# jrl-umi3218/jrl-walkgen

Hardware: NVIDIA B200
Metric: Kajita preview steps/s (batched; Herdt2010 QP solves/s reported under 'herdt') (higher is better)
Workload: dtype f64

## Files before the change

jrl_walkgen_b200/csrc/preview.cu:

```cuda
#include "wg_common.h"
#include <atomic>
#include <mutex>
#include <cstdlib>
#include <vector>
#include <cmath>
#include <algorithm>
#include <type_traits>

#define WG_HD __host__ __device__

namespace {

struct Mat {
  int n;
  double a[16];
  WG_HD double &operator()(int i, int j) { return a[i * n + j]; }
  WG_HD double operator()(int i, int j) const { return a[i * n + j]; }
};

WG_HD Mat mat_zero(int n)
{
  Mat C;
  C.n = n;
  for (int i = 0; i < 16; ++i) C.a[i] = 0.0;
// ... 229 lines not shown
constexpr int SCAN_LEVELS = 6;

struct PreviewConsts {
  double A[9], B[3], C[3], Kx[3], Ks;
  int NL, NLpad;
  double P[2][SCAN_LEVELS][16];
  double G[2][FIR_R][4], H[2][FIR_R][4];
  double RF0[FIR_R], RFN[FIR_R];
  double RV[FIR_R][4], RVN[FIR_R][4];
  double RW[FIR_R + 1][4];
  double RP[SCAN_LEVELS][16];
};
__constant__ PreviewConsts c_pc;
__constant__ double c_F[WG_PREVIEW_MAX_NL + 8];

namespace {
struct PreviewImage {
  PreviewConsts pc;
  double F[WG_PREVIEW_MAX_NL + 8];
};
std::mutex g_pv_mutex;
std::atomic<unsigned long long> g_pv_gen_counter{0};
unsigned long long g_pv_bound[64];

int preview_bind(wg_ctx *ctx)
{
  if (ctx->device < 0 || ctx->device >= 64) return WG_ERR_INVALID;
  if (g_pv_bound[ctx->device] == ctx->preview_gen) return WG_OK;
  const PreviewImage *im = reinterpret_cast<const PreviewImage *>(ctx->preview_image.data());
  WG_CUDA(ctx, cudaDeviceSynchronize());
  WG_CUDA(ctx, cudaMemcpyToSymbol(c_pc, &im->pc, sizeof im->pc));
  WG_CUDA(ctx, cudaMemcpyToSymbol(c_F, im->F, sizeof im->F));
  g_pv_bound[ctx->device] = ctx->preview_gen;
  return WG_OK;
}
}

constexpr int PV_MAX_CHUNKS = 16;

struct wg_preview_plan {
  wg_ctx *ctx;
  int B;
  int NL;
  int64_t total_samples, total_steps;
  int64_t *d_offsets;
  int *d_order;
  double *d_zmp, *d_state, *d_com, *d_zmpout, *d_add;
  int n_chunks;
  int chunk_first[PV_MAX_CHUNKS + 1];
  int64_t chunk_samp[PV_MAX_CHUNKS + 1];
  int *d_order_chunked;
  cudaStream_t up_stream, down_stream;
  cudaEvent_t ev_up[PV_MAX_CHUNKS], ev_k[PV_MAX_CHUNKS], ev_done;
};

__device__ __forceinline__ int pad9(int e) { return e + (e >> 3); }
__device__ __forceinline__ int swz8(int e) { return e ^ ((e >> 3) & 7); }

struct Axis {
  double x0, x1, x2, s;
};
template <bool SIM>
__device__ __forceinline__ double preview_tick(Axis &a, double f, double pk)
{
  double r = c_pc.Kx[0] * a.x0;
  r = fma(c_pc.Kx[1], a.x1, r);
  r = fma(c_pc.Kx[2], a.x2, r);
  const double u = fma(c_pc.Ks, a.s, -r) + f;
  const double n0 = fma(c_pc.A[2], a.x2, fma(c_pc.A[1], a.x1, a.x0));
  const double n1 = fma(c_pc.A[5], a.x2, a.x1);
  a.x0 = fma(u, c_pc.B[0], n0);
  a.x1 = fma(u, c_pc.B[1], n1);
  a.x2 = fma(u, c_pc.B[2], a.x2);
  const double z = fma(c_pc.C[2], a.x2, fma(c_pc.C[1], a.x1, c_pc.C[0] * a.x0));
  if (SIM) a.s += (pk - z);
  return z;
}

__device__ __forceinline__ Axis axis_zero()
{
  Axis a;
  a.x0 = a.x1 = a.x2 = a.s = 0.0;
  return a;
}
__device__ __forceinline__ void operator+=(Axis &a, const Axis &b)
{
  a.x0 += b.x0; a.x1 += b.x1; a.x2 += b.x2; a.s += b.s;
}
__device__ __forceinline__ void axpy(Axis &c, const double *g, double a)
{
  c.x0 = fma(g[0], a, c.x0); c.x1 = fma(g[1], a, c.x1);
  c.x2 = fma(g[2], a, c.x2); c.s = fma(g[3], a, c.s);
}
__device__ __forceinline__ Axis shfl_up(const Axis &a, int d)
{
  Axis r;
  r.x0 = __shfl_up_sync(0xffffffffu, a.x0, d); r.x1 = __shfl_up_sync(0xffffffffu, a.x1, d);
  r.x2 = __shfl_up_sync(0xffffffffu, a.x2, d); r.s = __shfl_up_sync(0xffffffffu, a.s, d);
  return r;
}
__device__ __forceinline__ Axis shfl_down(const Axis &a, int d)
{
  Axis r;
  r.x0 = __shfl_down_sync(0xffffffffu, a.x0, d); r.x1 = __shfl_down_sync(0xffffffffu, a.x1, d);
  r.x2 = __shfl_down_sync(0xffffffffu, a.x2, d); r.s = __shfl_down_sync(0xffffffffu, a.s, d);
  return r;
// ... 501 lines not shown
            if (ADD) {
              double q[12];
              ld32g(ga + 6 * r0, q[0], q[1], q[2], q[3], c32);
              ld32g(ga + 6 * r0 + 4, q[4], q[5], q[6], q[7], c32);
              ld32g(ga + 6 * r0 + 8, q[8], q[9], q[10], q[11], c32);
              a0 += q[0]; a1 += q[1]; a2 += q[2]; a3 += q[3]; a4 += q[4]; a5 += q[5];
              b0 += q[6]; b1 += q[7]; b2 += q[8]; b3 += q[9]; b4 += q[10]; b5 += q[11];
            }
            st32g(gc + 6 * r0, a0, a1, a2, a3, c32);
            st32g(gc + 6 * r0 + 4, a4, a5, b0, b1, c32);
            st32g(gc + 6 * r0 + 8, b2, b3, b4, b5, c32);
          }
          if (zmp) st32g(gz + 2 * r0, u0, u1, POS ? sx.x0 : zx1, POS ? sy.x0 : zy1, z32);
        } else if (k0 + r0 <= last) {
          const double zx0 = preview_tick<SIM>(sx, ax[r0], pk[r0].x);
          const double zy0 = preview_tick<SIM>(sy, ay[r0], pk[r0].y);
          if (com) {
            double a0 = sx.x0, a1 = sx.x1, a2 = sx.x2, a3 = sy.x0, a4 = sy.x1, a5 = sy.x2;
            if (ADD) {
              const double2 q0 = __ldg(reinterpret_cast<const double2 *>(ga + 6 * r0));
              const double2 q1 = __ldg(reinterpret_cast<const double2 *>(ga + 6 * r0) + 1);
              const double2 q2 = __ldg(reinterpret_cast<const double2 *>(ga + 6 * r0) + 2);
              a0 += q0.x; a1 += q0.y; a2 += q1.x; a3 += q1.y; a4 += q2.x; a5 += q2.y;
            }
            double2 *g2 = reinterpret_cast<double2 *>(gc + 6 * r0);
            g2[0] = make_double2(a0, a1); g2[1] = make_double2(a2, a3); g2[2] = make_double2(a4, a5);
          }
          if (zmp) *reinterpret_cast<double2 *>(gz + 2 * r0) = POS ? make_double2(sx.x0, sy.x0) : make_double2(zx0, zy0);
        }
      }
    }
    if (k0 <= last && last < k0 + FIR_R) store_state(s_carry, sx, sy);
    base += FIR_TILE;
    if (base >= CAP) base -= CAP;
  }
  __syncthreads();
  if (t < 8) state[8 * (size_t)b + t] = s_carry[t];
}

constexpr int RW_TILE = FIR_R * 32;
constexpr int RW_U = 5;

__device__ __forceinline__ void bulk_store(double *dst, unsigned src_smem, unsigned bytes)
{
  asm volatile("cp.async.bulk.global.shared::cta.bulk_group [%0], [%1], %2;\n" ::"l"(dst), "r"(src_smem), "r"(bytes) : "memory");
}
__device__ __forceinline__ bool elect_one()
{
  unsigned r;
  asm volatile("{\n .reg .pred p;\n elect.sync _|p, 0xffffffff;\n selp.u32 %0, 1, 0, p;\n}\n" : "=r"(r));
  return r != 0;
}

template <bool SIM, bool ADD = false, bool POS = false>
__global__ void __launch_bounds__(32, 10)
preview_rec_warp_kernel(const int *__restrict__ order, const int64_t *__restrict__ offsets,
                        const double2 *__restrict__ p, double *__restrict__ state, double *__restrict__ com,
                        double *__restrict__ zmp, const double *__restrict__ com_add, const double2 *__restrict__ Etab)
{
  constexpr unsigned FULL = 0xffffffffu;
  extern __shared__ double2 sp[];
  __shared__ double s_halo[8];
  __shared__ double s_carry[8];
  const int b = order[blockIdx.x];
  const int64_t o = offsets[b];
  const int L = (int)(offsets[b + 1] - o);
  const int NL = c_pc.NL, NLpad = c_pc.NLpad;
  const int nsteps = L - NL + 1;
  if (nsteps <= 0) return;
  const int lane = threadIdx.x;
  const int CAP = RW_TILE + NLpad;
  double2 *stage = sp + CAP + 25 * lane;
  if (lane < 8) s_carry[lane] = state[8 * (size_t)b + lane];
  const double(*Pm)[16] = c_pc.P[SIM ? 1 : 0];
  const double2 *src = p + o;
  for (int e = lane; e < CAP; e += 32) cp_async16(sp + swz8(e), src + (e < L ? e : 0), e < L ? 16u : 0u);
  cp_async_commit();
  int base = 0;

  for (int start = 0; start < nsteps; start += RW_TILE) {
    cp_async_wait_all();
    __syncwarp();
    int own0 = base + FIR_R * lane;
    if (own0 >= CAP) own0 -= CAP;

    {
      double h[8];
#pragma unroll
      for (int j = 0; j < 8; ++j) h[j] = 0.0;
      int hb = base + RW_TILE;
      if (hb >= CAP) hb -= CAP;
      for (int i0 = lane; i0 < NL; i0 += 32 * RW_U) {
        double2 e01[RW_U], e23[RW_U], q[RW_U];
#pragma unroll
        for (int u = 0; u < RW_U; ++u) {
          const int i = i0 + 32 * u;
          const bool in = i < NL;
          const int ii = in ? i : 0;
          ld32g(reinterpret_cast<const double *>(Etab + 2 * ii), e01[u].x, e01[u].y, e23[u].x, e23[u].y, true);
          int hi = hb + ii;
          if (hi >= CAP) hi -= CAP;
          q[u] = in ? sp[swz8(hi)] : make_double2(0.0, 0.0);
        }
#pragma unroll
        for (int u = 0; u < RW_U; ++u) {
          h[0] = fma(e01[u].x, q[u].x, h[0]); h[1] = fma(e01[u].y, q[u].x, h[1]);
          h[2] = fma(e23[u].x, q[u].x, h[2]); h[3] = fma(e23[u].y, q[u].x, h[3]);
          h[4] = fma(e01[u].x, q[u].y, h[4]); h[5] = fma(e01[u].y, q[u].y, h[5]);
          h[6] = fma(e23[u].x, q[u].y, h[6]); h[7] = fma(e23[u].y, q[u].y, h[7]);
        }
      }
      double k4[4], k2[2], k1;
      {
        const bool up = (lane & 16) != 0;
#pragma unroll
        for (int j = 0; j < 4; ++j) {
          const double send = up ? h[j] : h[4 + j];
          k4[j] = (up ? h[4 + j] : h[j]) + __shfl_xor_sync(FULL, send, 16);
        }
      }
      {
        const bool up = (lane & 8) != 0;
#pragma unroll
        for (int j = 0; j < 2; ++j) {
          const double send = up ? k4[j] : k4[2 + j];
          k2[j] = (up ? k4[2 + j] : k4[j]) + __shfl_xor_sync(FULL, send, 8);
        }
      }
      {
        const bool up = (lane & 4) != 0;
        const double send = up ? k2[0] : k2[1];
        k1 = (up ? k2[1] : k2[0]) + __shfl_xor_sync(FULL, send, 4);
      }
      k1 += __shfl_xor_sync(FULL, k1, 2);
      k1 += __shfl_xor_sync(FULL, k1, 1);
      if ((lane & 3) == 0) s_halo[((lane & 16) ? 4 : 0) + ((lane & 8) ? 2 : 0) + ((lane & 4) ? 1 : 0)] = k1;
    }

    double ax[FIR_R], ay[FIR_R];
    double2 pk[FIR_R];
    Axis bx, by;
    {
      const double2 *own = sp + own0;
      const int osw = (own0 >> 3) & 7;
      local_pass<SIM>([&](int j) { return own[j ^ osw]; }, [&](int i) { return sp[swz8(i)]; }, own0, NL, CAP, ax, ay, pk, bx, by);
    }
    __syncwarp();
    if (start + RW_TILE < nsteps) {
      const int first = start + CAP;
#pragma unroll
      for (int u = 0; u < FIR_R; ++u) {
        const int e = lane + 32 * u;
        int ri = base + e;
        if (ri >= CAP) ri -= CAP;
        const bool in = first + e < L;
        cp_async16(sp + swz8(ri), src + (in ? first + e : 0), in ? 16u : 0u);
      }
      cp_async_commit();
    }
    Axis ix, iy;
    load_pair(s_halo, ix, iy);
    if (lane == 31) {
      scan_combine(bx, c_pc.RP[0], ix);
      scan_combine(by, c_pc.RP[0], iy);
    }
    scan_down(bx, by, lane);
    {
      const Axis a = shfl_down(bx, 1), b = shfl_down(by, 1);
      if (lane != 31) { ix = a; iy = b; }
    }
    add_window(ax, ay, ix, iy);

    Axis cx, cy, inx, iny;
    local_aggregate<SIM>(ax, ay, pk, lane == 0, s_carry, Pm, cx, cy, inx, iny);
    scan_up(cx, cy, lane, Pm);
    Axis sx = shfl_up(cx, 1), sy = shfl_up(cy, 1);
    if (lane == 0) { sx = inx; sy = iny; }
    __syncwarp();
    const int k0 = start + FIR_R * lane;
    const int last = min(start + RW_TILE, nsteps) - 1;
    {
      double *gc = com ? com + 6 * (size_t)(o + k0) : nullptr;
      double *gz = zmp ? zmp + 2 * (size_t)(o + k0) : nullptr;
      const double *ga = ADD ? com_add + 6 * (size_t)(o + k0) : nullptr;
      const bool c32 = ((reinterpret_cast<uintptr_t>(gc) | (ADD ? reinterpret_cast<uintptr_t>(ga) : 0)) & 31) == 0;
      const bool z32 = (reinterpret_cast<uintptr_t>(gz) & 31) == 0;
      const bool bulk = com != nullptr;
      if (bulk) {
        asm volatile("cp.async.bulk.wait_group.read 0;\n" ::: "memory");
        __syncwarp();
      }
#pragma unroll
      for (int j = 0; j < FIR_R / 2; ++j) {
        const int r0 = 2 * j, r1 = 2 * j + 1;
        if (k0 + r1 <= last) {
          const double zx0 = preview_tick<SIM>(sx, ax[r0], pk[r0].x);
          const double zy0 = preview_tick<SIM>(sy, ay[r0], pk[r0].y);
          double a0 = sx.x0, a1 = sx.x1, a2 = sx.x2, a3 = sy.x0, a4 = sy.x1, a5 = sy.x2;
          const double u0 = POS ? sx.x0 : zx0, u1 = POS ? sy.x0 : zy0;
          const double zx1 = preview_tick<SIM>(sx, ax[r1], pk[r1].x);
          const double zy1 = preview_tick<SIM>(sy, ay[r1], pk[r1].y);
          if (com) {
            double b0 = sx.x0, b1 = sx.x1, b2 = sx.x2, b3 = sy.x0, b4 = sy.x1, b5 = sy.x2;
            if (ADD) {
              double q[12];
              ld32g(ga + 6 * r0, q[0], q[1], q[2], q[3], c32);
              ld32g(ga + 6 * r0 + 4, q[4], q[5], q[6], q[7], c32);
              ld32g(ga + 6 * r0 + 8, q[8], q[9], q[10], q[11], c32);
              a0 += q[0]; a1 += q[1]; a2 += q[2]; a3 += q[3]; a4 += q[4]; a5 += q[5];
              b0 += q[6]; b1 += q[7]; b2 += q[8]; b3 += q[9]; b4 += q[10]; b5 += q[11];
            }
            if (bulk) {
              double2 *sg = stage + 6 * j;
              sg[0] = make_double2(a0, a1); sg[1] = make_double2(a2, a3); sg[2] = make_double2(a4, a5);
              sg[3] = make_double2(b0, b1); sg[4] = make_double2(b2, b3); sg[5] = make_double2(b4, b5);
            } else {
              st32g(gc + 6 * r0, a0, a1, a2, a3, c32);
              st32g(gc + 6 * r0 + 4, a4, a5, b0, b1, c32);
              st32g(gc + 6 * r0 + 8, b2, b3, b4, b5, c32);
            }
          }
          if (zmp) st32g(gz + 2 * r0, u0, u1, POS ? sx.x0 : zx1, POS ? sy.x0 : zy1, z32);
        } else if (k0 + r0 <= last) {
          const double zx0 = preview_tick<SIM>(sx, ax[r0], pk[r0].x);
          const double zy0 = preview_tick<SIM>(sy, ay[r0], pk[r0].y);
          if (com) {
            double a0 = sx.x0, a1 = sx.x1, a2 = sx.x2, a3 = sy.x0, a4 = sy.x1, a5 = sy.x2;
            if (ADD) {
              const double2 q0 = __ldg(reinterpret_cast<const double2 *>(ga + 6 * r0));
              const double2 q1 = __ldg(reinterpret_cast<const double2 *>(ga + 6 * r0) + 1);
              const double2 q2 = __ldg(reinterpret_cast<const double2 *>(ga + 6 * r0) + 2);
              a0 += q0.x; a1 += q0.y; a2 += q1.x; a3 += q1.y; a4 += q2.x; a5 += q2.y;
            }
            double2 *g2 = reinterpret_cast<double2 *>(gc + 6 * r0);
            g2[0] = make_double2(a0, a1); g2[1] = make_double2(a2, a3); g2[2] = make_double2(a4, a5);
          }
          if (zmp) *reinterpret_cast<double2 *>(gz + 2 * r0) = POS ? make_double2(sx.x0, sy.x0) : make_double2(zx0, zy0);
        }
      }
      if (bulk) {
        asm volatile("fence.proxy.async.shared::cta;\n" ::: "memory");
        __syncwarp();
        if (elect_one()) {
          const int nt = last - start + 1;
          double *g = com + 6 * (size_t)(o + start);
          const unsigned sa = (unsigned)__cvta_generic_to_shared(sp + CAP);
          if (nt >= RW_TILE) {
#pragma unroll
            for (int i = 0; i < 32; ++i) bulk_store(g + 6 * FIR_R * i, sa + 400u * i, 96u * (FIR_R / 2));
          } else {
            for (int i = 0; i < 32 && FIR_R * i + 1 < nt; ++i)
              bulk_store(g + 6 * FIR_R * i, sa + 400u * i, 96u * (unsigned)min(FIR_R / 2, (nt - FIR_R * i) / 2));
          }
          asm volatile("cp.async.bulk.commit_group;\n" ::: "memory");
        }
      }
    }
    if (k0 <= last && last < k0 + FIR_R) store_state(s_carry, sx, sy);
    base += RW_TILE;
    if (base >= CAP) base -= CAP;
  }
  __syncwarp();
  asm volatile("cp.async.bulk.wait_group 0;\n" ::: "memory");
  if (lane < 8) state[8 * (size_t)b + lane] = s_carry[lane];
}

namespace {

void scan_matrices(const wg_preview_gains_t &g, bool sim, double (*P)[16], double (*G)[4], double (*H)[4])
{
  typedef long double LD;
  LD M[4][4];
  for (int j = 0; j < 4; ++j) {
    LD x[3] = {0, 0, 0}, s = 0;
    if (j < 3) x[j] = 1; else s = 1;
    const LD u = (LD)g.Ks * s - ((LD)g.Kx[0] * x[0] + (LD)g.Kx[1] * x[1] + (LD)g.Kx[2] * x[2]);
    LD n[3];
    for (int i = 0; i < 3; ++i)
      n[i] = (LD)g.A[3 * i] * x[0] + (LD)g.A[3 * i + 1] * x[1] + (LD)g.A[3 * i + 2] * x[2] + (LD)g.B[i] * u;
    const LD z = (LD)g.C[0] * n[0] + (LD)g.C[1] * n[1] + (LD)g.C[2] * n[2];
    for (int i = 0; i < 3; ++i) M[i][j] = n[i];
    M[3][j] = sim ? s - z : s;
  }
  auto square = [](LD X[4][4]) {
    LD Y[4][4];
    for (int i = 0; i < 4; ++i)
      for (int j = 0; j < 4; ++j) {
        LD a = 0;
        for (int k = 0; k < 4; ++k) a += X[i][k] * X[k][j];
        Y[i][j] = a;
      }
    std::memcpy(X, Y, sizeof Y);
  };
  if (G && H) {
    LD g4[4], h4[4] = {0, 0, 0, 0};
    LD zb = 0;
    for (int i = 0; i < 3; ++i) { g4[i] = (LD)g.B[i]; zb += (LD)g.C[i] * (LD)g.B[i]; }
    g4[3] = sim ? -zb : (LD)0;
    h4[3] = sim ? (LD)1 : (LD)0;
    for (int r = FIR_R - 1; r >= 0; --r) {
      for (int i = 0; i < 4; ++i) { G[r][i] = (double)g4[i]; H[r][i] = (double)h4[i]; }
      LD gn[4], hn[4];
      for (int i = 0; i < 4; ++i) {
        gn[i] = 0; hn[i] = 0;
        for (int k = 0; k < 4; ++k) { gn[i] += M[i][k] * g4[k]; hn[i] += M[i][k] * h4[k]; }
      }
      std::memcpy(g4, gn, sizeof gn); std::memcpy(h4, hn, sizeof hn);
    }
  }
  for (int r = 1; r < FIR_R; r <<= 1) square(M);
  for (int l = 0; l < SCAN_LEVELS; ++l) {
    for (int i = 0; i < 4; ++i)
      for (int j = 0; j < 4; ++j) P[l][4 * i + j] = (double)M[i][j];
    square(M);
  }
}

// ... 117 lines not shown
    std::memcpy(Pl, P8, sizeof Pl);
    for (int l = 0; l < SCAN_LEVELS; ++l) {
      for (int i = 0; i < 4; ++i) for (int j = 0; j < 4; ++j) pc.RP[l][4 * i + j] = (double)Pl[i][j];
      mul(Pl, Pl, Pl);
    }
    LD Pm[4][4];
    for (int i = 0; i < 4; ++i) for (int j = 0; j < 4; ++j) Pm[i][j] = (i == j) ? 1 : 0;
    double *lp = tables.data() + (size_t)NLpad * 4;
    for (int m = 0; m < 32; ++m) {
      for (int i = 0; i < 4; ++i) for (int j = 0; j < 4; ++j) lp[16 * m + 4 * i + j] = (double)Pm[i][j];
      mul(P8, Pm, Pm);
    }
  }
  return (double)(res / tot);
}

}

template <class... P, class... A>
static int preview_launch(wg_ctx *ctx, void (*kern)(P...), int count, int threads, size_t smem, const char *too_large,
                          A... args)
{
  if (smem > 96 * 1024) return wg_fail(ctx, WG_ERR_INVALID, too_large);
  std::lock_guard<std::mutex> lock(g_pv_mutex);
  { const int rc = preview_bind(ctx); if (rc != WG_OK) return rc; }
  WG_SMEM_ATTR(ctx, kern, smem);
  wg_prof_start(ctx, WG_K_PREVIEW_FUSED);
  kern<<<count, threads, smem, ctx->stream>>>(args...);
  wg_prof_stop(ctx);
  WG_LAUNCHED(ctx);
  return WG_OK;
}

template <bool SIM, bool ADD, bool POS>
static int preview_launch_variant(wg_ctx *ctx, wg_preview_plan *pl, bool recursive, int shape, const int *d_order, int count,
                                  const double2 *pz, double *d_state, double *d_com, double *d_zmpout, const double *d_com_add)
{
  const int NLpad = (pl->NL + FIR_R - 1) / FIR_R * FIR_R;
  const int64_t *off = pl->d_offsets;
  if (!recursive) {
    auto smem = [&](int threads) {
      const int span = FIR_R * threads + NLpad;
      return sizeof(double2) * std::max<size_t>((size_t)(span + (span >> 3) + 2), (size_t)(threads / 32) * 320);
    };
    const char *msg = "preview window too large for the FIR tile";
    switch (shape) {
    case 1: return preview_launch(ctx, preview_fused_kernel<SIM, 128, 4, ADD, POS>, count, 128, smem(128), msg, d_order, off, pz, d_state, d_com, d_zmpout, d_com_add);
    case 2: return preview_launch(ctx, preview_fused_kernel<SIM, 32, 16, ADD, POS>, count, 32, smem(32), msg, d_order, off, pz, d_state, d_com, d_zmpout, d_com_add);
    default: return preview_launch(ctx, preview_fused_kernel<SIM, 64, 8, ADD, POS>, count, 64, smem(64), msg, d_order, off, pz, d_state, d_com, d_zmpout, d_com_add);
    }
  }
  const double2 *E = reinterpret_cast<const double2 *>(ctx->preview_rec_dev);
  const char *msg = "preview window too large for the tile";
  if (shape == 2)
    return preview_launch(ctx, preview_rec_warp_kernel<SIM, ADD, POS>, count, 32, sizeof(double2) * (size_t)(RW_TILE + NLpad + 25 * 32),
                          msg, d_order, off, pz, d_state, d_com, d_zmpout, d_com_add, E);
  auto smem = [&](int threads) {
    const int cap = 2 * FIR_R * threads + NLpad;
    return sizeof(double2) * (size_t)(cap + (cap >> 3) + 2);
  };
  const double2 *lp = E + 2 * (size_t)NLpad;
  switch (shape) {
  case 1: return preview_launch(ctx, preview_rec_kernel<SIM, 128, 4, ADD, POS>, count, 128, smem(128), msg, d_order, off, pz, d_state, d_com, d_zmpout, d_com_add, E, lp);
  case 3: return preview_launch(ctx, preview_rec_kernel<SIM, 256, 2, ADD, POS>, count, 256, smem(256), msg, d_order, off, pz, d_state, d_com, d_zmpout, d_com_add, E, lp);
  default: return preview_launch(ctx, preview_rec_kernel<SIM, 64, 8, ADD, POS>, count, 64, smem(64), msg, d_order, off, pz, d_state, d_com, d_zmpout, d_com_add, E, lp);
  }
}

extern "C" {

int wg_preview_set_gains(wg_ctx *ctx, const wg_preview_gains_t *g)
{
  if (!ctx || !g || g->NL <= 0 || g->NL > WG_PREVIEW_MAX_NL) return WG_ERR_INVALID;
  wg_device_guard guard(ctx->device);
  static_assert((FIR_R & (FIR_R - 1)) == 0, "FIR_R must be a power of two");
  ctx->preview_image.assign(sizeof(PreviewImage), 0);
  PreviewImage *im = reinterpret_cast<PreviewImage *>(ctx->preview_image.data());
  PreviewConsts &pc = im->pc;
  std::memcpy(pc.A, g->A, sizeof pc.A);
  std::memcpy(pc.B, g->B, sizeof pc.B);
  std::memcpy(pc.C, g->C, sizeof pc.C);
  std::memcpy(pc.Kx, g->Kx, sizeof pc.Kx);
  pc.Ks = g->Ks;
  pc.NL = g->NL;
  pc.NLpad = (g->NL + FIR_R - 1) / FIR_R * FIR_R;
  scan_matrices(*g, false, pc.P[0], pc.G[0], pc.H[0]);
  scan_matrices(*g, true, pc.P[1], pc.G[1], pc.H[1]);
  std::copy(g->F, g->F + g->NL, im->F);
  {
    std::vector<double> tables;
    ctx->preview_rec_residual = rec_setup(*g, pc, tables);
    ctx->preview_rec_ok = ctx->preview_rec_residual >= 0.0 && ctx->preview_rec_residual <= WG_PREVIEW_REC_TOL;
    if (ctx->preview_rec_dev) { WG_CUDA(ctx, cudaStreamSynchronize(ctx->stream)); cudaFree(ctx->preview_rec_dev); ctx->preview_rec_dev = nullptr; }
    if (ctx->preview_rec_ok) {
      WG_CUDA(ctx, cudaMalloc(&ctx->preview_rec_dev, sizeof(double) * tables.size()));
      WG_CUDA(ctx, cudaMemcpy(ctx->preview_rec_dev, tables.data(), sizeof(double) * tables.size(), cudaMemcpyHostToDevice));
    }
  }
  ctx->preview_gains = *g;
  ctx->preview_gen = ++g_pv_gen_counter;
  ctx->preview_ready = true;
  return WG_OK;
}

double wg_preview_sum_fit(const wg_preview_gains_t *g)
{
  if (!g || g->NL <= 0 || g->NL > WG_PREVIEW_MAX_NL) return -1.0;
  PreviewConsts pc;
  std::vector<double> tables;
// ... 38 lines not shown
{
  if (!ctx) return WG_ERR_INVALID;
  if (!ctx->preview_ready) return wg_fail(ctx, WG_ERR_NOT_READY, "wg_preview_set_gains not called");
  if (mode_in_use)
    *mode_in_use = (ctx->preview_sum_mode != WG_PREVIEW_SUM_DIRECT && ctx->preview_rec_ok) ? WG_PREVIEW_SUM_RECURSIVE : WG_PREVIEW_SUM_DIRECT;
  if (fit_residual) *fit_residual = ctx->preview_rec_residual;
  return WG_OK;
}

int wg_preview_plan_create(wg_ctx *ctx, int B, const int64_t *offsets, wg_preview_plan **out)
{
  if (!ctx || !out || B < 0 || (B > 0 && !offsets)) return WG_ERR_INVALID;
  if (!ctx->preview_ready) return wg_fail(ctx, WG_ERR_NOT_READY, "wg_preview_set_gains not called");
  wg_device_guard guard(ctx->device);
  *out = nullptr;
  const int NL = ctx->preview_gains.NL;
  if (B > 0 && offsets[0] != 0) return wg_fail(ctx, WG_ERR_INVALID, "offsets[0] must be 0");
  int64_t total_steps = 0;
  std::vector<int> order(B);
  for (int b = 0; b < B; ++b) {
    const int64_t L = offsets[b + 1] - offsets[b];
    if (L < 0 || L > 0x3fffffff) return wg_fail(ctx, WG_ERR_INVALID, "offsets must be non-decreasing");
    if (L >= NL) total_steps += L - NL + 1;
    order[b] = b;
  }
  std::stable_sort(order.begin(), order.end(), [&](int a, int b) {
    return offsets[a + 1] - offsets[a] > offsets[b + 1] - offsets[b];
  });
  wg_preview_plan *pl = new (std::nothrow) wg_preview_plan();
  if (!pl) return WG_ERR_ALLOC;
  std::memset(pl, 0, sizeof *pl);
  pl->ctx = ctx; pl->B = B; pl->NL = NL;
  pl->total_samples = B > 0 ? offsets[B] : 0;
  pl->total_steps = total_steps;
  pl->n_chunks = std::max(1, std::min(PV_MAX_CHUNKS, B / 8));
  {
    const int64_t total = B > 0 ? offsets[B] : 0;
    int b = 0;
    pl->chunk_first[0] = 0;
    for (int c = 1; c < pl->n_chunks; ++c) {
      const int64_t target = total * c / pl->n_chunks;
      while (b < B && offsets[b] < target) ++b;
      pl->chunk_first[c] = std::max(b, pl->chunk_first[c - 1]);
    }
    pl->chunk_first[pl->n_chunks] = B;
    for (int c = 0; c <= pl->n_chunks; ++c) pl->chunk_samp[c] = B > 0 ? offsets[pl->chunk_first[c]] : 0;
  }
  std::vector<int> order_chunked(B);
  for (int b = 0; b < B; ++b) order_chunked[b] = b;
  for (int c = 0; c < pl->n_chunks; ++c)
    std::stable_sort(order_chunked.begin() + pl->chunk_first[c], order_chunked.begin() + pl->chunk_first[c + 1], [&](int a, int b) {
      return offsets[a + 1] - offsets[a] > offsets[b + 1] - offsets[b];
    });
  cudaError_t e = cudaMalloc(&pl->d_offsets, sizeof(int64_t) * (B + 1));
  if (e == cudaSuccess) e = cudaMalloc(&pl->d_order, sizeof(int) * std::max(1, B));
  if (e == cudaSuccess) e = cudaMalloc(&pl->d_order_chunked, sizeof(int) * std::max(1, B));
  if (e == cudaSuccess && B > 0)
    e = cudaMemcpyAsync(pl->d_order_chunked, order_chunked.data(), sizeof(int) * B, cudaMemcpyHostToDevice, ctx->stream);
  if (e == cudaSuccess) e = cudaStreamCreateWithFlags(&pl->up_stream, cudaStreamNonBlocking);
  if (e == cudaSuccess) e = cudaStreamCreateWithFlags(&pl->down_stream, cudaStreamNonBlocking);
  for (int c = 0; c < PV_MAX_CHUNKS && e == cudaSuccess; ++c) {
    e = cudaEventCreateWithFlags(&pl->ev_up[c], cudaEventDisableTiming);
    if (e == cudaSuccess) e = cudaEventCreateWithFlags(&pl->ev_k[c], cudaEventDisableTiming);
  }
  if (e == cudaSuccess) e = cudaEventCreateWithFlags(&pl->ev_done, cudaEventDisableTiming);
  if (e == cudaSuccess && B > 0)
    e = cudaMemcpyAsync(pl->d_offsets, offsets, sizeof(int64_t) * (B + 1), cudaMemcpyHostToDevice, ctx->stream);
  if (e == cudaSuccess && B > 0)
    e = cudaMemcpyAsync(pl->d_order, order.data(), sizeof(int) * B, cudaMemcpyHostToDevice, ctx->stream);
  if (e == cudaSuccess) e = cudaStreamSynchronize(ctx->stream);
  if (e != cudaSuccess) {
    wg_fail(ctx, WG_ERR_CUDA, "wg_preview_plan_create", e);
    wg_preview_plan_destroy(pl);
    return WG_ERR_CUDA;
  }
  *out = pl;
  return WG_OK;
}

int wg_preview_plan_destroy(wg_preview_plan *pl)
{
  if (!pl) return WG_OK;
  wg_device_guard guard(pl->ctx->device);
  cudaStreamSynchronize(pl->ctx->stream);
  if (pl->up_stream) { cudaStreamSynchronize(pl->up_stream); cudaStreamDestroy(pl->up_stream); }
  if (pl->down_stream) { cudaStreamSynchronize(pl->down_stream); cudaStreamDestroy(pl->down_stream); }
  for (int c = 0; c < PV_MAX_CHUNKS; ++c) { if (pl->ev_up[c]) cudaEventDestroy(pl->ev_up[c]); if (pl->ev_k[c]) cudaEventDestroy(pl->ev_k[c]); }
  if (pl->ev_done) cudaEventDestroy(pl->ev_done);
  cudaFree(pl->d_offsets); cudaFree(pl->d_order); cudaFree(pl->d_order_chunked);
  cudaFree(pl->d_zmp); cudaFree(pl->d_state); cudaFree(pl->d_com); cudaFree(pl->d_zmpout); cudaFree(pl->d_add);
  delete pl;
  return WG_OK;
}

int wgi_preview_plan_set_offsets(wg_preview_plan *pl, const int64_t *offsets_host)
{
  wg_ctx *ctx = pl->ctx;
  int64_t total_steps = 0;
  for (int b = 0; b < pl->B; ++b) {
    const int64_t L = offsets_host[b + 1] - offsets_host[b];
    if (L >= pl->NL) total_steps += L - pl->NL + 1;
  }
  pl->total_samples = pl->B > 0 ? offsets_host[pl->B] : 0;
  pl->total_steps = total_steps;
  if (pl->B > 0)
    WG_CUDA(ctx, cudaMemcpyAsync(pl->d_offsets, offsets_host, sizeof(int64_t) * (pl->B + 1), cudaMemcpyHostToDevice, ctx->stream));
  return WG_OK;
}

int64_t wg_preview_plan_total_steps(const wg_preview_plan *pl) { return pl ? pl->total_steps : 0; }
int64_t wg_preview_plan_total_samples(const wg_preview_plan *pl) { return pl ? pl->total_samples : 0; }

int wgi_preview_launch_range(wg_ctx *ctx, wg_preview_plan *pl, const int *d_order, int count, const double *d_zmp,
                            double *d_state, double *d_com, double *d_zmpout, int simulation, const double *d_com_add,
                            int pos_only)
{
  if (pl->total_steps == 0 || count <= 0) return WG_OK;
  static int forced = -2;
  if (forced == -2) {
    const char *e = getenv("WG_PREVIEW_SHAPE");
    forced = e ? atoi(e) : -1;
  }
  const bool recursive = ctx->preview_sum_mode != WG_PREVIEW_SUM_DIRECT && ctx->preview_rec_ok;
  int shape = forced >= 0 ? forced : ctx->preview_cta_shape >= 0 ? ctx->preview_cta_shape : !recursive ? 0 : count >= 1792 ? 2 : count >= 768 ? 1 : 3;
  if (shape == 3) {
    const int NLpad = (pl->NL + FIR_R - 1) / FIR_R * FIR_R, cap = 2 * FIR_R * 256 + NLpad;
    if (!recursive || sizeof(double2) * (size_t)(cap + (cap >> 3) + 2) > 96 * 1024) shape = 1;
  }
  if (ctx->preview_sum_mode == WG_PREVIEW_SUM_RECURSIVE && !ctx->preview_rec_ok)
    return wg_fail(ctx, WG_ERR_INVALID, "WG_PREVIEW_SUM_RECURSIVE: the window weights of this context are not of the form w' L^i v");
  const double2 *pz = reinterpret_cast<const double2 *>(d_zmp);
  auto launch = [&](auto sim, auto add, auto pos) {
    return preview_launch_variant<sim, add, pos>(ctx, pl, recursive, shape, d_order, count, pz, d_state, pos ? nullptr : d_com,
                                                 d_zmpout, add ? d_com_add : nullptr);
  };
  const std::true_type T{};
  const std::false_type F{};
  if (pos_only) return simulation ? launch(T, F, T) : launch(F, F, T);
  if (d_com_add && d_com) return launch(T, T, F);
  return simulation ? launch(T, F, F) : launch(F, F, F);
}

// ... 212 lines not shown
```

Before: 50.64 billion.

## Make warp preview kernel persistent with atomic ticket work-stealing across walks

Converts the one-warp-per-walk preview kernel into a persistent kernel launched with as many blocks as fit resident on the GPU. Each warp takes walk indices from a global atomic ticket counter and prefetches the next walk's first window while finishing the current one. The tile body is factored into a helper with refill and carry callbacks. This is meant to cut per-block launch and scheduling overhead and to overlap the next walk's load with the current tail. The cost is an atomic per walk and a monotonically growing ticket counter kept on the host.

```diff
diff --git a/jrl_walkgen_b200/csrc/preview.cu b/jrl_walkgen_b200/csrc/preview.cu
--- a/jrl_walkgen_b200/csrc/preview.cu
+++ b/jrl_walkgen_b200/csrc/preview.cu
@@ -305,6 +305,9 @@
   int *d_order_chunked;
   cudaStream_t up_stream, down_stream;
   cudaEvent_t ev_up[PV_MAX_CHUNKS], ev_k[PV_MAX_CHUNKS], ev_done;
+  unsigned long long *d_next;
+  unsigned long long tickets;
+  int resident;
 };
 
 __device__ __forceinline__ int pad9(int e) { return e + (e >> 3); }
@@ -912,217 +915,262 @@
   return r != 0;
 }
 
+template <bool SIM, bool ADD, bool POS, class Refill, class CarryIn, class CarryOut>
+__device__ __forceinline__ void rec_warp_tile(double2 *sp, double *s_halo, int lane, int CAP, int base, int start, int nsteps,
+                                              int64_t o, double *com, double *zmp, const double *com_add, const double2 *Etab,
+                                              Refill refill, CarryIn carry_in, CarryOut carry_out)
+{
+  constexpr unsigned FULL = 0xffffffffu;
+  const int NL = c_pc.NL;
+  const double(*Pm)[16] = c_pc.P[SIM ? 1 : 0];
+  double2 *stage = sp + CAP + 25 * lane;
+  int own0 = base + FIR_R * lane;
+  if (own0 >= CAP) own0 -= CAP;
+
+  {
+    double h[8];
+#pragma unroll
+    for (int j = 0; j < 8; ++j) h[j] = 0.0;
+    int hb = base + RW_TILE;
+    if (hb >= CAP) hb -= CAP;
+    for (int i0 = lane; i0 < NL; i0 += 32 * RW_U) {
+      double2 e01[RW_U], e23[RW_U], q[RW_U];
+#pragma unroll
+      for (int u = 0; u < RW_U; ++u) {
+        const int i = i0 + 32 * u;
+        const bool in = i < NL;
+        const int ii = in ? i : 0;
+        ld32g(reinterpret_cast<const double *>(Etab + 2 * ii), e01[u].x, e01[u].y, e23[u].x, e23[u].y, true);
+        int hi = hb + ii;
+        if (hi >= CAP) hi -= CAP;
+        q[u] = in ? sp[swz8(hi)] : make_double2(0.0, 0.0);
+      }
+#pragma unroll
+      for (int u = 0; u < RW_U; ++u) {
+        h[0] = fma(e01[u].x, q[u].x, h[0]); h[1] = fma(e01[u].y, q[u].x, h[1]);
+        h[2] = fma(e23[u].x, q[u].x, h[2]); h[3] = fma(e23[u].y, q[u].x, h[3]);
+        h[4] = fma(e01[u].x, q[u].y, h[4]); h[5] = fma(e01[u].y, q[u].y, h[5]);
+        h[6] = fma(e23[u].x, q[u].y, h[6]); h[7] = fma(e23[u].y, q[u].y, h[7]);
+      }
+    }
+    double k4[4], k2[2], k1;
+    {
+      const bool up = (lane & 16) != 0;
+#pragma unroll
+      for (int j = 0; j < 4; ++j) {
+        const double send = up ? h[j] : h[4 + j];
+        k4[j] = (up ? h[4 + j] : h[j]) + __shfl_xor_sync(FULL, send, 16);
+      }
+    }
+    {
+      const bool up = (lane & 8) != 0;
+#pragma unroll
+      for (int j = 0; j < 2; ++j) {
+        const double send = up ? k4[j] : k4[2 + j];
+        k2[j] = (up ? k4[2 + j] : k4[j]) + __shfl_xor_sync(FULL, send, 8);
+      }
+    }
+    {
+      const bool up = (lane & 4) != 0;
+      const double send = up ? k2[0] : k2[1];
+      k1 = (up ? k2[1] : k2[0]) + __shfl_xor_sync(FULL, send, 4);
+    }
+    k1 += __shfl_xor_sync(FULL, k1, 2);
+    k1 += __shfl_xor_sync(FULL, k1, 1);
+    if ((lane & 3) == 0) s_halo[((lane & 16) ? 4 : 0) + ((lane & 8) ? 2 : 0) + ((lane & 4) ? 1 : 0)] = k1;
+  }
+
+  double ax[FIR_R], ay[FIR_R];
+  double2 pk[FIR_R];
+  Axis bx, by;
+  {
+    const double2 *own = sp + own0;
+    const int osw = (own0 >> 3) & 7;
+    local_pass<SIM>([&](int j) { return own[j ^ osw]; }, [&](int i) { return sp[swz8(i)]; }, own0, NL, CAP, ax, ay, pk, bx, by);
+  }
+  __syncwarp();
+  refill();
+  Axis ix, iy;
+  load_pair(s_halo, ix, iy);
+  if (lane == 31) {
+    scan_combine(bx, c_pc.RP[0], ix);
+    scan_combine(by, c_pc.RP[0], iy);
+  }
+  scan_down(bx, by, lane);
+  {
+    const Axis a = shfl_down(bx, 1), b = shfl_down(by, 1);
+    if (lane != 31) { ix = a; iy = b; }
+  }
+  add_window(ax, ay, ix, iy);
+
+  Axis cx, cy, inx, iny;
+  {
+    double q[8];
+    const double *cin = carry_in(q);
+    local_aggregate<SIM>(ax, ay, pk, lane == 0, cin, Pm, cx, cy, inx, iny);
+  }
+  scan_up(cx, cy, lane, Pm);
+  Axis sx = shfl_up(cx, 1), sy = shfl_up(cy, 1);
+  if (lane == 0) { sx = inx; sy = iny; }
+  __syncwarp();
+  const int k0 = start + FIR_R * lane;
+  const int last = min(start + RW_TILE, nsteps) - 1;
+  {
+    double *gc = com ? com + 6 * (size_t)(o + k0) : nullptr;
+    double *gz = zmp ? zmp + 2 * (size_t)(o + k0) : nullptr;
+    const double *ga = ADD ? com_add + 6 * (size_t)(o + k0) : nullptr;
+    const bool c32 = ((reinterpret_cast<uintptr_t>(gc) | (ADD ? reinterpret_cast<uintptr_t>(ga) : 0)) & 31) == 0;
+    const bool z32 = (reinterpret_cast<uintptr_t>(gz) & 31) == 0;
+    const bool bulk = com != nullptr;
+    if (bulk) {
+      asm volatile("cp.async.bulk.wait_group.read 0;\n" ::: "memory");
+      __syncwarp();
+    }
+#pragma unroll
+    for (int j = 0; j < FIR_R / 2; ++j) {
+      const int r0 = 2 * j, r1 = 2 * j + 1;
+      if (k0 + r1 <= last) {
+        const double zx0 = preview_tick<SIM>(sx, ax[r0], pk[r0].x);
+        const double zy0 = preview_tick<SIM>(sy, ay[r0], pk[r0].y);
+        double a0 = sx.x0, a1 = sx.x1, a2 = sx.x2, a3 = sy.x0, a4 = sy.x1, a5 = sy.x2;
+        const double u0 = POS ? sx.x0 : zx0, u1 = POS ? sy.x0 : zy0;
+        const double zx1 = preview_tick<SIM>(sx, ax[r1], pk[r1].x);
+        const double zy1 = preview_tick<SIM>(sy, ay[r1], pk[r1].y);
+        if (com) {
+          double b0 = sx.x0, b1 = sx.x1, b2 = sx.x2, b3 = sy.x0, b4 = sy.x1, b5 = sy.x2;
+          if (ADD) {
+            double q[12];
+            ld32g(ga + 6 * r0, q[0], q[1], q[2], q[3], c32);
+            ld32g(ga + 6 * r0 + 4, q[4], q[5], q[6], q[7], c32);
+            ld32g(ga + 6 * r0 + 8, q[8], q[9], q[10], q[11], c32);
+            a0 += q[0]; a1 += q[1]; a2 += q[2]; a3 += q[3]; a4 += q[4]; a5 += q[5];
+            b0 += q[6]; b1 += q[7]; b2 += q[8]; b3 += q[9]; b4 += q[10]; b5 += q[11];
+          }
+          if (bulk) {
+            double2 *sg = stage + 6 * j;
+            sg[0] = make_double2(a0, a1); sg[1] = make_double2(a2, a3); sg[2] = make_double2(a4, a5);
+            sg[3] = make_double2(b0, b1); sg[4] = make_double2(b2, b3); sg[5] = make_double2(b4, b5);
+          } else {
+            st32g(gc + 6 * r0, a0, a1, a2, a3, c32);
+            st32g(gc + 6 * r0 + 4, a4, a5, b0, b1, c32);
+            st32g(gc + 6 * r0 + 8, b2, b3, b4, b5, c32);
+          }
+        }
+        if (zmp) st32g(gz + 2 * r0, u0, u1, POS ? sx.x0 : zx1, POS ? sy.x0 : zy1, z32);
+      } else if (k0 + r0 <= last) {
+        const double zx0 = preview_tick<SIM>(sx, ax[r0], pk[r0].x);
+        const double zy0 = preview_tick<SIM>(sy, ay[r0], pk[r0].y);
+        if (com) {
+          double a0 = sx.x0, a1 = sx.x1, a2 = sx.x2, a3 = sy.x0, a4 = sy.x1, a5 = sy.x2;
+          if (ADD) {
+            const double2 q0 = __ldg(reinterpret_cast<const double2 *>(ga + 6 * r0));
+            const double2 q1 = __ldg(reinterpret_cast<const double2 *>(ga + 6 * r0) + 1);
+            const double2 q2 = __ldg(reinterpret_cast<const double2 *>(ga + 6 * r0) + 2);
+            a0 += q0.x; a1 += q0.y; a2 += q1.x; a3 += q1.y; a4 += q2.x; a5 += q2.y;
+          }
+          double2 *g2 = reinterpret_cast<double2 *>(gc + 6 * r0);
+          g2[0] = make_double2(a0, a1); g2[1] = make_double2(a2, a3); g2[2] = make_double2(a4, a5);
+        }
+        if (zmp) *reinterpret_cast<double2 *>(gz + 2 * r0) = POS ? make_double2(sx.x0, sy.x0) : make_double2(zx0, zy0);
+      }
+    }
+    if (bulk) {
+      asm volatile("fence.proxy.async.shared::cta;\n" ::: "memory");
+      __syncwarp();
+      if (elect_one()) {
+        const int nt = last - start + 1;
+        double *g = com + 6 * (size_t)(o + start);
+        const unsigned sa = (unsigned)__cvta_generic_to_shared(sp + CAP);
+        if (nt >= RW_TILE) {
+#pragma unroll
+          for (int i = 0; i < 32; ++i) bulk_store(g + 6 * FIR_R * i, sa + 400u * i, 96u * (FIR_R / 2));
+        } else {
+          for (int i = 0; i < 32 && FIR_R * i + 1 < nt; ++i)
+            bulk_store(g + 6 * FIR_R * i, sa + 400u * i, 96u * (unsigned)min(FIR_R / 2, (nt - FIR_R * i) / 2));
+        }
+        asm volatile("cp.async.bulk.commit_group;\n" ::: "memory");
+      }
+    }
+  }
+  if (k0 <= last && last < k0 + FIR_R) carry_out(sx, sy);
+}
+
 template <bool SIM, bool ADD = false, bool POS = false>
 __global__ void __launch_bounds__(32, 10)
-preview_rec_warp_kernel(const int *__restrict__ order, const int64_t *__restrict__ offsets,
-                        const double2 *__restrict__ p, double *__restrict__ state, double *__restrict__ com,
-                        double *__restrict__ zmp, const double *__restrict__ com_add, const double2 *__restrict__ Etab)
+preview_rec_warp_kernel(const int *__restrict__ order, int count, unsigned long long *next, unsigned long long ticket0,
+                        const int64_t *__restrict__ offsets, const double2 *__restrict__ p, double *__restrict__ state,
+                        double *__restrict__ com, double *__restrict__ zmp, const double *__restrict__ com_add,
+                        const double2 *__restrict__ Etab)
 {
   constexpr unsigned FULL = 0xffffffffu;
   extern __shared__ double2 sp[];
   __shared__ double s_halo[8];
   __shared__ double s_carry[8];
-  const int b = order[blockIdx.x];
-  const int64_t o = offsets[b];
-  const int L = (int)(offsets[b + 1] - o);
-  const int NL = c_pc.NL, NLpad = c_pc.NLpad;
-  const int nsteps = L - NL + 1;
-  if (nsteps <= 0) return;
   const int lane = threadIdx.x;
-  const int CAP = RW_TILE + NLpad;
-  double2 *stage = sp + CAP + 25 * lane;
-  if (lane < 8) s_carry[lane] = state[8 * (size_t)b + lane];
-  const double(*Pm)[16] = c_pc.P[SIM ? 1 : 0];
-  const double2 *src = p + o;
-  for (int e = lane; e < CAP; e += 32) cp_async16(sp + swz8(e), src + (e < L ? e : 0), e < L ? 16u : 0u);
-  cp_async_commit();
-  int base = 0;
-
-  for (int start = 0; start < nsteps; start += RW_TILE) {
-    cp_async_wait_all();
+  const int NL = c_pc.NL;
+  const int CAP = RW_TILE + c_pc.NLpad;
+  unsigned tk = 0;
+  auto walk_of = [&](unsigned t) {
+    while (true) {
+      const unsigned i = __shfl_sync(FULL, t, 0) - (unsigned)ticket0;
+      if (i >= (unsigned)count) return -1;
+      const int b = order[i];
+      if (offsets[b + 1] - offsets[b] >= NL) return b;
+      if (lane == 0) t = (unsigned)atomicAdd(next, 1ull);
+    }
+  };
+  auto first_window = [&](int b) {
+    const int64_t o = offsets[b];
+    const int L = (int)(offsets[b + 1] - o);
+    for (int e = lane; e < CAP; e += 32) cp_async16(sp + swz8(e), p + o + (e < L ? e : 0), e < L ? 16u : 0u);
+    cp_async_commit();
+  };
+  if (lane == 0) tk = (unsigned)atomicAdd(next, 1ull);
+  int b = walk_of(tk);
+  if (b < 0) return;
+  first_window(b);
+  while (b >= 0) {
+    if (lane == 0) tk = (unsigned)atomicAdd(next, 1ull);
+    int nb = -1;
+    const int64_t o = offsets[b];
+    const int L = (int)(offsets[b + 1] - o);
+    const int nsteps = L - NL + 1;
+    const double2 *src = p + o;
+    if (lane < 8) s_carry[lane] = state[8 * (size_t)b + lane];
+    int base = 0;
+    for (int start = 0; start < nsteps; start += RW_TILE) {
+      cp_async_wait_all();
+      __syncwarp();
+      rec_warp_tile<SIM, ADD, POS>(
+          sp, s_halo, lane, CAP, base, start, nsteps, o, com, zmp, com_add, Etab,
+          [&] {
+            if (start + RW_TILE < nsteps) {
+              const int first = start + CAP;
+#pragma unroll
+              for (int u = 0; u < FIR_R; ++u) {
+                const int e = lane + 32 * u;
+                int ri = base + e;
+                if (ri >= CAP) ri -= CAP;
+                const bool in = first + e < L;
+                cp_async16(sp + swz8(ri), src + (in ? first + e : 0), in ? 16u : 0u);
+              }
+              cp_async_commit();
+            } else {
+              nb = walk_of(tk);
+              if (nb >= 0) first_window(nb);
+            }
+          },
+          [&](double *) -> const double * { return s_carry; },
+          [&](const Axis &x, const Axis &y) { store_state(s_carry, x, y); });
+      base += RW_TILE;
+      if (base >= CAP) base -= CAP;
+    }
     __syncwarp();
-    int own0 = base + FIR_R * lane;
-    if (own0 >= CAP) own0 -= CAP;
-
-    {
-      double h[8];
-#pragma unroll
-      for (int j = 0; j < 8; ++j) h[j] = 0.0;
-      int hb = base + RW_TILE;
-      if (hb >= CAP) hb -= CAP;
-      for (int i0 = lane; i0 < NL; i0 += 32 * RW_U) {
-        double2 e01[RW_U], e23[RW_U], q[RW_U];
-#pragma unroll
-        for (int u = 0; u < RW_U; ++u) {
-          const int i = i0 + 32 * u;
-          const bool in = i < NL;
-          const int ii = in ? i : 0;
-          ld32g(reinterpret_cast<const double *>(Etab + 2 * ii), e01[u].x, e01[u].y, e23[u].x, e23[u].y, true);
-          int hi = hb + ii;
-          if (hi >= CAP) hi -= CAP;
-          q[u] = in ? sp[swz8(hi)] : make_double2(0.0, 0.0);
-        }
-#pragma unroll
-        for (int u = 0; u < RW_U; ++u) {
-          h[0] = fma(e01[u].x, q[u].x, h[0]); h[1] = fma(e01[u].y, q[u].x, h[1]);
-          h[2] = fma(e23[u].x, q[u].x, h[2]); h[3] = fma(e23[u].y, q[u].x, h[3]);
-          h[4] = fma(e01[u].x, q[u].y, h[4]); h[5] = fma(e01[u].y, q[u].y, h[5]);
-          h[6] = fma(e23[u].x, q[u].y, h[6]); h[7] = fma(e23[u].y, q[u].y, h[7]);
-        }
-      }
-      double k4[4], k2[2], k1;
-      {
-        const bool up = (lane & 16) != 0;
-#pragma unroll
-        for (int j = 0; j < 4; ++j) {
-          const double send = up ? h[j] : h[4 + j];
-          k4[j] = (up ? h[4 + j] : h[j]) + __shfl_xor_sync(FULL, send, 16);
-        }
-      }
-      {
-        const bool up = (lane & 8) != 0;
-#pragma unroll
-        for (int j = 0; j < 2; ++j) {
-          const double send = up ? k4[j] : k4[2 + j];
-          k2[j] = (up ? k4[2 + j] : k4[j]) + __shfl_xor_sync(FULL, send, 8);
-        }
-      }
-      {
-        const bool up = (lane & 4) != 0;
-        const double send = up ? k2[0] : k2[1];
-        k1 = (up ? k2[1] : k2[0]) + __shfl_xor_sync(FULL, send, 4);
-      }
-      k1 += __shfl_xor_sync(FULL, k1, 2);
-      k1 += __shfl_xor_sync(FULL, k1, 1);
-      if ((lane & 3) == 0) s_halo[((lane & 16) ? 4 : 0) + ((lane & 8) ? 2 : 0) + ((lane & 4) ? 1 : 0)] = k1;
-    }
-
-    double ax[FIR_R], ay[FIR_R];
-    double2 pk[FIR_R];
-    Axis bx, by;
-    {
-      const double2 *own = sp + own0;
-      const int osw = (own0 >> 3) & 7;
-      local_pass<SIM>([&](int j) { return own[j ^ osw]; }, [&](int i) { return sp[swz8(i)]; }, own0, NL, CAP, ax, ay, pk, bx, by);
-    }
+    if (lane < 8) state[8 * (size_t)b + lane] = s_carry[lane];
     __syncwarp();
-    if (start + RW_TILE < nsteps) {
-      const int first = start + CAP;
-#pragma unroll
-      for (int u = 0; u < FIR_R; ++u) {
-        const int e = lane + 32 * u;
-        int ri = base + e;
-        if (ri >= CAP) ri -= CAP;
-        const bool in = first + e < L;
-        cp_async16(sp + swz8(ri), src + (in ? first + e : 0), in ? 16u : 0u);
-      }
-      cp_async_commit();
-    }
-    Axis ix, iy;
-    load_pair(s_halo, ix, iy);
-    if (lane == 31) {
-      scan_combine(bx, c_pc.RP[0], ix);
-      scan_combine(by, c_pc.RP[0], iy);
-    }
-    scan_down(bx, by, lane);
-    {
-      const Axis a = shfl_down(bx, 1), b = shfl_down(by, 1);
-      if (lane != 31) { ix = a; iy = b; }
-    }
-    add_window(ax, ay, ix, iy);
-
-    Axis cx, cy, inx, iny;
-    local_aggregate<SIM>(ax, ay, pk, lane == 0, s_carry, Pm, cx, cy, inx, iny);
-    scan_up(cx, cy, lane, Pm);
-    Axis sx = shfl_up(cx, 1), sy = shfl_up(cy, 1);
-    if (lane == 0) { sx = inx; sy = iny; }
-    __syncwarp();
-    const int k0 = start + FIR_R * lane;
-    const int last = min(start + RW_TILE, nsteps) - 1;
-    {
-      double *gc = com ? com + 6 * (size_t)(o + k0) : nullptr;
-      double *gz = zmp ? zmp + 2 * (size_t)(o + k0) : nullptr;
-      const double *ga = ADD ? com_add + 6 * (size_t)(o + k0) : nullptr;
-      const bool c32 = ((reinterpret_cast<uintptr_t>(gc) | (ADD ? reinterpret_cast<uintptr_t>(ga) : 0)) & 31) == 0;
-      const bool z32 = (reinterpret_cast<uintptr_t>(gz) & 31) == 0;
-      const bool bulk = com != nullptr;
-      if (bulk) {
-        asm volatile("cp.async.bulk.wait_group.read 0;\n" ::: "memory");
-        __syncwarp();
-      }
-#pragma unroll
-      for (int j = 0; j < FIR_R / 2; ++j) {
-        const int r0 = 2 * j, r1 = 2 * j + 1;
-        if (k0 + r1 <= last) {
-          const double zx0 = preview_tick<SIM>(sx, ax[r0], pk[r0].x);
-          const double zy0 = preview_tick<SIM>(sy, ay[r0], pk[r0].y);
-          double a0 = sx.x0, a1 = sx.x1, a2 = sx.x2, a3 = sy.x0, a4 = sy.x1, a5 = sy.x2;
-          const double u0 = POS ? sx.x0 : zx0, u1 = POS ? sy.x0 : zy0;
-          const double zx1 = preview_tick<SIM>(sx, ax[r1], pk[r1].x);
-          const double zy1 = preview_tick<SIM>(sy, ay[r1], pk[r1].y);
-          if (com) {
-            double b0 = sx.x0, b1 = sx.x1, b2 = sx.x2, b3 = sy.x0, b4 = sy.x1, b5 = sy.x2;
-            if (ADD) {
-              double q[12];
-              ld32g(ga + 6 * r0, q[0], q[1], q[2], q[3], c32);
-              ld32g(ga + 6 * r0 + 4, q[4], q[5], q[6], q[7], c32);
-              ld32g(ga + 6 * r0 + 8, q[8], q[9], q[10], q[11], c32);
-              a0 += q[0]; a1 += q[1]; a2 += q[2]; a3 += q[3]; a4 += q[4]; a5 += q[5];
-              b0 += q[6]; b1 += q[7]; b2 += q[8]; b3 += q[9]; b4 += q[10]; b5 += q[11];
-            }
-            if (bulk) {
-              double2 *sg = stage + 6 * j;
-              sg[0] = make_double2(a0, a1); sg[1] = make_double2(a2, a3); sg[2] = make_double2(a4, a5);
-              sg[3] = make_double2(b0, b1); sg[4] = make_double2(b2, b3); sg[5] = make_double2(b4, b5);
-            } else {
-              st32g(gc + 6 * r0, a0, a1, a2, a3, c32);
-              st32g(gc + 6 * r0 + 4, a4, a5, b0, b1, c32);
-              st32g(gc + 6 * r0 + 8, b2, b3, b4, b5, c32);
-            }
-          }
-          if (zmp) st32g(gz + 2 * r0, u0, u1, POS ? sx.x0 : zx1, POS ? sy.x0 : zy1, z32);
-        } else if (k0 + r0 <= last) {
-          const double zx0 = preview_tick<SIM>(sx, ax[r0], pk[r0].x);
-          const double zy0 = preview_tick<SIM>(sy, ay[r0], pk[r0].y);
-          if (com) {
-            double a0 = sx.x0, a1 = sx.x1, a2 = sx.x2, a3 = sy.x0, a4 = sy.x1, a5 = sy.x2;
-            if (ADD) {
-              const double2 q0 = __ldg(reinterpret_cast<const double2 *>(ga + 6 * r0));
-              const double2 q1 = __ldg(reinterpret_cast<const double2 *>(ga + 6 * r0) + 1);
-              const double2 q2 = __ldg(reinterpret_cast<const double2 *>(ga + 6 * r0) + 2);
-              a0 += q0.x; a1 += q0.y; a2 += q1.x; a3 += q1.y; a4 += q2.x; a5 += q2.y;
-            }
-            double2 *g2 = reinterpret_cast<double2 *>(gc + 6 * r0);
-            g2[0] = make_double2(a0, a1); g2[1] = make_double2(a2, a3); g2[2] = make_double2(a4, a5);
-          }
-          if (zmp) *reinterpret_cast<double2 *>(gz + 2 * r0) = POS ? make_double2(sx.x0, sy.x0) : make_double2(zx0, zy0);
-        }
-      }
-      if (bulk) {
-        asm volatile("fence.proxy.async.shared::cta;\n" ::: "memory");
-        __syncwarp();
-        if (elect_one()) {
-          const int nt = last - start + 1;
-          double *g = com + 6 * (size_t)(o + start);
-          const unsigned sa = (unsigned)__cvta_generic_to_shared(sp + CAP);
-          if (nt >= RW_TILE) {
-#pragma unroll
-            for (int i = 0; i < 32; ++i) bulk_store(g + 6 * FIR_R * i, sa + 400u * i, 96u * (FIR_R / 2));
-          } else {
-            for (int i = 0; i < 32 && FIR_R * i + 1 < nt; ++i)
-              bulk_store(g + 6 * FIR_R * i, sa + 400u * i, 96u * (unsigned)min(FIR_R / 2, (nt - FIR_R * i) / 2));
-          }
-          asm volatile("cp.async.bulk.commit_group;\n" ::: "memory");
-        }
-      }
-    }
-    if (k0 <= last && last < k0 + FIR_R) store_state(s_carry, sx, sy);
-    base += RW_TILE;
-    if (base >= CAP) base -= CAP;
-  }
-  __syncwarp();
+    b = nb;
+  }
   asm volatile("cp.async.bulk.wait_group 0;\n" ::: "memory");
-  if (lane < 8) state[8 * (size_t)b + lane] = s_carry[lane];
 }
 
 namespace {
@@ -1346,9 +1394,13 @@
   }
   const double2 *E = reinterpret_cast<const double2 *>(ctx->preview_rec_dev);
   const char *msg = "preview window too large for the tile";
-  if (shape == 2)
-    return preview_launch(ctx, preview_rec_warp_kernel<SIM, ADD, POS>, count, 32, sizeof(double2) * (size_t)(RW_TILE + NLpad + 25 * 32),
-                          msg, d_order, off, pz, d_state, d_com, d_zmpout, d_com_add, E);
+  if (shape == 2) {
+    const int grid = std::min(count, pl->resident);
+    const int rc = preview_launch(ctx, preview_rec_warp_kernel<SIM, ADD, POS>, grid, 32, sizeof(double2) * (size_t)(RW_TILE + NLpad + 25 * 32),
+                                  msg, d_order, count, pl->d_next, pl->tickets, off, pz, d_state, d_com, d_zmpout, d_com_add, E);
+    if (rc == WG_OK) pl->tickets += (unsigned long long)count + grid;
+    return rc;
+  }
   auto smem = [&](int threads) {
     const int cap = 2 * FIR_R * threads + NLpad;
     return sizeof(double2) * (size_t)(cap + (cap >> 3) + 2);
@@ -1493,7 +1545,17 @@
     std::stable_sort(order_chunked.begin() + pl->chunk_first[c], order_chunked.begin() + pl->chunk_first[c + 1], [&](int a, int b) {
       return offsets[a + 1] - offsets[a] > offsets[b + 1] - offsets[b];
     });
-  cudaError_t e = cudaMalloc(&pl->d_offsets, sizeof(int64_t) * (B + 1));
+  const size_t smem_warp = sizeof(double2) * (size_t)(RW_TILE + (NL + FIR_R - 1) / FIR_R * FIR_R + 25 * 32);
+  {
+    const int rc = wgi_smem_attr(ctx, reinterpret_cast<const void *>(preview_rec_warp_kernel<true>), smem_warp);
+    if (rc != WG_OK) { wg_preview_plan_destroy(pl); return rc; }
+  }
+  int per_sm = 0;
+  cudaError_t e = cudaOccupancyMaxActiveBlocksPerMultiprocessor(&per_sm, preview_rec_warp_kernel<true>, 32, smem_warp);
+  pl->resident = std::max(1, per_sm) * std::max(1, ctx->sm_count);
+  if (e == cudaSuccess) e = cudaMalloc(&pl->d_next, sizeof(unsigned long long));
+  if (e == cudaSuccess) e = cudaMemsetAsync(pl->d_next, 0, sizeof(unsigned long long), ctx->stream);
+  if (e == cudaSuccess) e = cudaMalloc(&pl->d_offsets, sizeof(int64_t) * (B + 1));
   if (e == cudaSuccess) e = cudaMalloc(&pl->d_order, sizeof(int) * std::max(1, B));
   if (e == cudaSuccess) e = cudaMalloc(&pl->d_order_chunked, sizeof(int) * std::max(1, B));
   if (e == cudaSuccess && B > 0)
@@ -1528,7 +1590,7 @@
   if (pl->down_stream) { cudaStreamSynchronize(pl->down_stream); cudaStreamDestroy(pl->down_stream); }
   for (int c = 0; c < PV_MAX_CHUNKS; ++c) { if (pl->ev_up[c]) cudaEventDestroy(pl->ev_up[c]); if (pl->ev_k[c]) cudaEventDestroy(pl->ev_k[c]); }
   if (pl->ev_done) cudaEventDestroy(pl->ev_done);
-  cudaFree(pl->d_offsets); cudaFree(pl->d_order); cudaFree(pl->d_order_chunked);
+  cudaFree(pl->d_offsets); cudaFree(pl->d_order); cudaFree(pl->d_order_chunked); cudaFree(pl->d_next);
   cudaFree(pl->d_zmp); cudaFree(pl->d_state); cudaFree(pl->d_com); cudaFree(pl->d_zmpout); cudaFree(pl->d_add);
   delete pl;
   return WG_OK;
```

Result: slower. 46.05 billion, median of 6 (-9.1%).
